# WeiZhang1988/YDORBSLAM

Measured on AMD Instinct MI355X. Metric: ORB extract+match Mkeypoints/sec, higher is better.
Workload: dtype u8

## Files before the change

ydorbslam_amd/csrc/ba_kernels.hip.h:

```cpp
#pragma once
#include <hip/hip_runtime.h>
#include <stdint.h>
#include "g2o_math.hip.h"

#pragma clang fp contract(off)

namespace ydorb {
namespace ba {

using g2o::R; using g2o::V3; using g2o::Q4;
using g2o::add; using g2o::cross; using g2o::scale; using g2o::qrot; using g2o::qmul; using g2o::qToR; using g2o::rToQ; using g2o::qnormalize;
using g2o::huber; using g2o::block_sums; using g2o::block_sum1; using g2o::dense_solve; using g2o::lambda_init; using g2o::lm_judge;

struct Cam { R fx, fy, cx, cy, bf; };

struct EdgeSoA {
  const int* pose;
  const int* pidx;
  const int* pt;
  const R* meas;
  const R* info;
  const uint8_t* robust;
  int n;
};
// ... 271 lines not shown

__device__ __forceinline__ int pair_bucket(int i1, int i2) { return i2 * (i2 + 1) / 2 + i1; }

__global__ __launch_bounds__(256) void k_pair_count(EdgeSoA Ed, const int* __restrict__ ptStart, int nL, int* __restrict__ cnt) {
  const int l = blockIdx.x * 256 + threadIdx.x;
  if (l >= nL) return;
  for (int a = ptStart[l]; a < ptStart[l + 1]; a++) {
    const int i1 = Ed.pidx[a];
    if (i1 < 0) continue;
    for (int b = a; b < ptStart[l + 1]; b++) {
      const int i2 = Ed.pidx[b];
      if (i2 >= 0) atomicAdd(&cnt[pair_bucket(i1, i2)], 1);
    }
  }
}
__global__ __launch_bounds__(256) void k_excl_scan(const int* __restrict__ in, int n, int* __restrict__ out) {
  __shared__ int wsum[4];
  __shared__ int carryS;
  const int lane = threadIdx.x & 63, wv = threadIdx.x >> 6;
  if (threadIdx.x == 0) carryS = 0;
  __syncthreads();
  for (int c0 = 0; c0 < n; c0 += 256) {
    const int i = c0 + threadIdx.x;
    const int v = i < n ? in[i] : 0;
    int x = v;
#pragma unroll
    for (int d = 1; d < 64; d <<= 1) { const int y = __shfl_up(x, d, 64); if (lane >= d) x += y; }
    if (lane == 63) wsum[wv] = x;
    __syncthreads();
    int off = carryS;
    for (int j = 0; j < wv; j++) off += wsum[j];
    if (i < n) out[i] = off + x - v;
    __syncthreads();
    if (threadIdx.x == 0) carryS += wsum[0] + wsum[1] + wsum[2] + wsum[3];
    __syncthreads();
  }
  if (threadIdx.x == 0) out[n] = carryS;
}
__global__ __launch_bounds__(256) void k_pair_fill(EdgeSoA Ed, const int* __restrict__ ptStart, int nL, int* __restrict__ cursor,
                                                   int2* __restrict__ items) {
  const int l = blockIdx.x * 256 + threadIdx.x;
  if (l >= nL) return;
  for (int a = ptStart[l]; a < ptStart[l + 1]; a++) {
    const int i1 = Ed.pidx[a];
    if (i1 < 0) continue;
    for (int b = a; b < ptStart[l + 1]; b++) {
      const int i2 = Ed.pidx[b];
      if (i2 >= 0) items[atomicAdd(&cursor[pair_bucket(i1, i2)], 1)] = make_int2(a, b);
    }
  }
}
constexpr int kSortCap = 2048;
// ... 857 lines not shown
```

ydorbslam_amd/csrc/ba_solver.hip:

```cpp
#include <hip/hip_runtime.h>
#include <chrono>

#include <algorithm>
#include <string>
#include <thread>
#include <atomic>
#include <cmath>
#include <cstring>
#include <limits>
#include <mutex>
#include <numeric>
#include <optional>
#include <vector>

#include "../../include/ydorb/c_api.h"
#include "ba_kernels.hip.h"
#include "ba_pairs.h"
#include "ba_skyline.hip.h"
#include "host_buffers.h"
#include "lm_schedule.h"
#include "ydorb_host.h"

using namespace ydorb;
using namespace ydorb::ba;

namespace {

enum { PH_ERR = 0, PH_BUILD, PH_SCHUR, PH_SOLVE, PH_UPDATE, PH_COUNT };

struct Sys {
  std::vector<int> act; int nL = 0, nPf = 0, Ea = 0, n = 0, nb = 0, nBlkE = 0, nBuckets = 0, nPoseEdges = 0; size_t nItems = 0;
  bool sky = false;
  sky::Plan plan;
  size_t envDoubles() const { return 36 * (size_t)plan.envBlocks; }
};
static_assert(bapairs::kDenseMaxRows == kCholSolveMaxN, "ba_pairs.h states the dense limit for the host-only plan");

struct StatePtrs { double *poses[2], *pts[2]; };
size_t layState(int K, int NP, void* base, StatePtrs& st) {
  Carve a(base);
  for (int i = 0; i < 2; i++) { a.take(st.poses[i], (size_t)7 * K); a.take(st.pts[i], (size_t)3 * NP); }
  return a.L.bytes;
}

struct SkyPtrs { int *pairRow, *pairI1, *pairI2, *perm, *first, *colRows; long long *pairDst, *rowOff, *colStart, *colBlk; };
struct UpPtrs { int *ePose, *ePidx, *ePt, *eLm, *ptStart, *poseStart, *ptOf, *poseEdges, *poseOf; double *eMeas, *eInfo; uint8_t* eRobust; SkyPtrs k; };
size_t layUp(const Sys& Y, void* base, UpPtrs& u) {
  Carve a(base);
  const size_t Ea = Y.Ea;
  a.take(u.ePose, Ea); a.take(u.ePidx, Ea); a.take(u.ePt, Ea); a.take(u.eLm, Ea); a.take(u.eMeas, 3 * Ea); a.take(u.eInfo, Ea); a.take(u.eRobust, Ea);
  a.take(u.ptStart, Y.nL + 1); a.take(u.poseStart, Y.nPf + 1); a.take(u.ptOf, Y.nL); a.take(u.poseEdges, Y.nPoseEdges); a.take(u.poseOf, Y.nPf);
  u.k = SkyPtrs{};
  if (Y.sky) {
    const size_t nB = Y.nBuckets, nF = Y.nPf, nCol = Y.plan.colRows.size();
    a.take(u.k.pairRow, nF + 1); a.take(u.k.pairI1, nB); a.take(u.k.pairI2, nB); a.take(u.k.pairDst, nB); a.take(u.k.perm, nF); a.take(u.k.first, nF);
    a.take(u.k.rowOff, nF + 1); a.take(u.k.colStart, nF + 1); a.take(u.k.colRows, nCol); a.take(u.k.colBlk, nCol);
  }
  return a.L.bytes;
}

struct WorkPtrs {
  double *eInfo0, *err, *partial, *Hll, *bl, *Hpl, *BD, *Hpp, *S, *diagInv, *diagL, *Dinv, *db, *xp, *xl, *yv, *skyW, *scal;
  uint8_t* eOutlier;
  int *status, *pairCnt, *pairStart, *pairCursor;
  int2 *pairA, *pairB;
  double* bp(const Sys& Y) const { return Hpp + (size_t)36 * Y.nPf; }
// ... 15 lines not shown
struct PosePtrs { int *start, *inl, *trials; double *poses, *X, *meas, *info, *err, *chi; uint8_t *flags, *outlier; };
size_t layPose(int n, size_t E, void* base, PosePtrs& q) {
  Carve a(base);
  a.take(q.start, n + 1); a.take(q.poses, (size_t)7 * n); a.take(q.X, 3 * E); a.take(q.meas, 3 * E); a.take(q.info, E);
  a.take(q.err, 3 * E); a.take(q.flags, E); a.take(q.outlier, E); a.take(q.inl, n); a.take(q.chi, (size_t)4 * n); a.take(q.trials, n);
  return a.L.bytes;
}

struct SolveMem {
  int device = -1;
  hipStream_t stream = nullptr;
  Mem state, up, work;
  StatePtrs st{};
  UpPtrs u{};
  WorkPtrs w{};
  PinnedMem hStage;
  int stage(size_t bytes) { return bytes <= hStage.cap ? YDORB_OK : hStage.alloc(bytes + bytes / 4 + 4096); }
  void releaseBuffers() { for (Mem* m : {&state, &up, &work, static_cast<Mem*>(&hStage)}) m->release(); }
};

struct Ctx {
  SolveMem mem;
  Mem pose;
  hipEvent_t ev[2 * PH_COUNT + 2]{};
  PinnedMem hPin;
  void releaseBuffers() { mem.releaseBuffers(); pose.release(); }
};
constexpr int kCtxPool = 8;
std::mutex g_mu[16][kCtxPool];
Ctx g_ctx[16][kCtxPool];
std::mutex g_pick;

// ... 12 lines not shown
    HIPCHK(hipStreamCreateWithFlags(&c.mem.stream, hipStreamNonBlocking));
    for (auto& e : c.ev) HIPCHK(hipEventCreate(&e));
    return c.hPin.alloc(sizeof(double) * 16);
  };
  if (!c.mem.stream && init() != YDORB_OK) return nullptr;
  return &c;
}

struct Run {
  SolveMem* c;
  const YdBaProblem* P;
  const YdBaOptions* O;
  YdBaResult* res;
  int cur = 0;
  bool noRobust = false;
  Cam cam;
  bool phaseTimes = false;
  double phaseMs[PH_COUNT] = {0, 0, 0, 0, 0};
  bool pending[PH_COUNT] = {false, false, false, false, false};
  Sys sys;
  hipEvent_t* ev = nullptr;
  double* hPin = nullptr;
  LmSchedule lm;
  const YdBaSolverOptions* SO = nullptr;
  YdBaSolverInfo* info = nullptr;
  bool stopped() const { return LmSchedule::raised(P->stop); }
};

int tooWideForSolve(int n) {
  set_error("reduced camera system of %d rows is wider than the solve kernel's LDS (max %d)", n, kCholSolveMaxN);
// ... 37 lines not shown
}

int allreduce(Run& R_, void* d_buf, int64_t count, int op) {
  const YdBaOptions* O = R_.O;
  if (!O->allreduce || O->world <= 1) return YDORB_OK;
  if (count > O->comm_doubles || !O->d_comm_buf) { set_error("BA comm buffer too small (%lld doubles needed)", (long long)count); return YDORB_ERR_CAPACITY; }
  HIPCHK(hipMemcpyAsync(O->d_comm_buf, d_buf, sizeof(double) * count, hipMemcpyDeviceToDevice, R_.c->stream));
  HIPCHK(hipStreamSynchronize(R_.c->stream));
  if (O->allreduce(O->allreduce_user, O->d_comm_buf, count, op) != 0) { set_error("BA all-reduce callback failed"); return YDORB_ERR_HIP; }
  HIPCHK(hipMemcpyAsync(d_buf, O->d_comm_buf, sizeof(double) * count, hipMemcpyDeviceToDevice, R_.c->stream));
  return YDORB_OK;
}

static bool g_trace = getenv("YDORB_BA_TRACE") != nullptr && getenv("YDORB_BA_TRACE")[0] == '1';
static std::chrono::steady_clock::time_point g_t0;
static void trace(const char* what) {
  if (!g_trace) return;
  fprintf(stderr, "[ba %8.3f ms] %s\n", std::chrono::duration<double, std::milli>(std::chrono::steady_clock::now() - g_t0).count(), what);
}

struct PhaseTimer {
  Run& r; int ph; hipEvent_t a, b; bool on;
  PhaseTimer(Run& r_, int ph_) : r(r_), ph(ph_), a(r_.ev[2 * ph_]), b(r_.ev[2 * ph_ + 1]), on(r_.phaseTimes) {
    if (!on) return;
    collect(r_, ph_);
    (void)hipEventRecord(a, r.c->stream);
  }
  void stop() { if (on) { (void)hipEventRecord(b, r.c->stream); on = false; r.pending[ph] = true; } }
  static void collect(Run& r_, int ph_) {
    if (!r_.pending[ph_]) return;
    float ms = 0;
    if (hipEventSynchronize(r_.ev[2 * ph_ + 1]) == hipSuccess && hipEventElapsedTime(&ms, r_.ev[2 * ph_], r_.ev[2 * ph_ + 1]) == hipSuccess)
      r_.phaseMs[ph_] += ms;
    r_.pending[ph_] = false;
  }
};

int prepareStage(Run& R_, bool reuse) {
  SolveMem& c = *R_.c;
  const YdBaProblem& P = *R_.P;
  const YdBaOptions& O = *R_.O;
  hipStream_t s = c.stream;
  const int K = P.n_poses, NP = P.n_points, E = P.n_edges;
  trace("optimize: begin");
  Sys& Y = R_.sys;
  auto prepare = [&]() -> int {
    std::vector<int> act;
    for (int e = 0; e < E; e++) act.push_back(e);
    if (act.empty()) { Y.Ea = 0; return YDORB_OK; }
    std::vector<int> poseIdx(K, -1), ptIdx(NP, -1), poseOf, ptOf;
    {
      std::vector<uint8_t> pu(K, 0), qu(NP, 0);
      for (int e : act) { pu[P.edge_pose[e]] = 1; qu[P.edge_point[e]] = 1; }
      for (int k = 0; k < K; k++) if (pu[k] && !P.pose_fixed[k]) { poseIdx[k] = (int)poseOf.size(); poseOf.push_back(k); }
      for (int p = 0; p < NP; p++) if (qu[p]) { ptIdx[p] = (int)ptOf.size(); ptOf.push_back(p); }
    }
    const int nL = (int)ptOf.size(), Ea = (int)act.size();
    if (O.world > 1) {
      poseOf.clear();
      for (int k = 0; k < K; k++) { poseIdx[k] = -1; if (!P.pose_fixed[k]) { poseIdx[k] = (int)poseOf.size(); poseOf.push_back(k); } }
    }
    const int nPf = (int)poseOf.size();
    {
      std::vector<int> start(nL + 1, 0), sorted(Ea);
      for (int e : act) start[ptIdx[P.edge_point[e]] + 1]++;
      for (int l = 0; l < nL; l++) start[l + 1] += start[l];
      std::vector<int> fill(start.begin(), start.end() - 1);
      for (int e : act) sorted[fill[ptIdx[P.edge_point[e]]]++] = e;
      auto after = [&](int x, int y) {
        const int px = poseIdx[P.edge_pose[x]], py = poseIdx[P.edge_pose[y]];
        return px != py ? px > py : P.edge_pose[x] > P.edge_pose[y];
      };
      for (int l = 0; l < nL; l++)
        for (int a = start[l] + 1; a < start[l + 1]; a++) {
          const int e = sorted[a];
          int b = a - 1;
          while (b >= start[l] && after(sorted[b], e)) { sorted[b + 1] = sorted[b]; b--; }
          sorted[b + 1] = e;
          if (b >= start[l] && P.edge_pose[sorted[b]] == P.edge_pose[e]) {
            set_error("edges %d and %d are both the observation of point %d by pose %d", sorted[b], e, P.edge_point[e], P.edge_pose[e]);
            return YDORB_ERR_INVALID_ARG;
          }
        }
      act.swap(sorted);
    }
    std::vector<int> hPose(Ea), hPidx(Ea), hPt(Ea), hLm(Ea), hPtStart(nL + 1, 0), hPoseStart(nPf + 1, 0), hPoseEdges;
    std::vector<double> hMeas((size_t)3 * Ea), hInfo(Ea);
    std::vector<uint8_t> hRobust(Ea);
    for (int i = 0; i < Ea; i++) {
      const int e = act[i];
      hPose[i] = P.edge_pose[e]; hPidx[i] = poseIdx[P.edge_pose[e]]; hPt[i] = P.edge_point[e]; hLm[i] = ptIdx[P.edge_point[e]];
      for (int d = 0; d < 3; d++) hMeas[3 * i + d] = P.edge_meas[3 * e + d];
      hInfo[i] = P.edge_inv_sigma2[e];
      hRobust[i] = R_.noRobust ? 0 : 1;
      hPtStart[hLm[i] + 1]++;
      if (hPidx[i] >= 0) hPoseStart[hPidx[i] + 1]++;
    }
    for (int l = 0; l < nL; l++) hPtStart[l + 1] += hPtStart[l];
    for (int i = 0; i < nPf; i++) hPoseStart[i + 1] += hPoseStart[i];
    hPoseEdges.resize(hPoseStart[nPf]);
    {
      std::vector<int> fill(hPoseStart.begin(), hPoseStart.end() - 1);
      for (int i = 0; i < Ea; i++) if (hPidx[i] >= 0) hPoseEdges[fill[hPidx[i]]++] = i;
    }
    Sys Z;
    Z.nL = nL; Z.nPf = nPf; Z.Ea = Ea; Z.nPoseEdges = (int)hPoseEdges.size();
    Z.n = std::max(NB, (6 * nPf + NB - 1) / NB * NB); Z.nb = Z.n / NB;
    Z.nBlkE = (Ea + 255) / 256;
    Z.nBuckets = (int)std::min<long long>((long long)nPf * (nPf + 1) / 2, std::numeric_limits<int>::max());
    for (int l = 0; l < nL; l++) {
      size_t m = 0;
      for (int i = hPtStart[l]; i < hPtStart[l + 1]; i++) m += hPidx[i] >= 0;
      Z.nItems += m * (m + 1) / 2;
    }
    bapairs::PairList pairs;
    std::vector<int64_t> pairDst;
    {
      int rc = chooseSolver(R_.SO, O.world, nPf, [&] { return bapairs::buildPairs(nPf, nL, hPtStart.data(), hPidx.data()); }, true, pairs, Z.plan, Z.sky, R_.info);
      if (rc) return rc;
      if (Z.sky) {
        Z.n = 6 * nPf; Z.nb = 0; Z.nBuckets = (int)pairs.buckets();
        pairDst = bapairs::bucketDestinations(pairs, Z.plan);
      }
    }
    trace("optimize: host ordering done");
    const size_t upBytes = layUp(Z, nullptr, c.u);
    int rc;
    if ((rc = c.stage(upBytes)) || (rc = c.up.ensure(upBytes)) || (rc = c.work.ensure(layWork(Z, nullptr, c.w)))) return rc;
    layUp(Z, c.up.p, c.u);
    layWork(Z, c.work.p, c.w);
    const UpPtrs& u = c.u;
    const WorkPtrs& w = c.w;
    {
      auto up = [&](const void* dst, const void* src, size_t bytes) {
        if (bytes) memcpy(c.hStage.as<uint8_t>() + (static_cast<const uint8_t*>(dst) - c.up.as<uint8_t>()), src, bytes);
      };
      auto upv = [&](const auto* dst, const auto& vec) { up(dst, vec.data(), sizeof(vec[0]) * vec.size()); };
      upv(u.ePose, hPose); upv(u.ePidx, hPidx); upv(u.ePt, hPt); upv(u.eLm, hLm); upv(u.eMeas, hMeas); upv(u.eInfo, hInfo);
      upv(u.eRobust, hRobust); upv(u.ptStart, hPtStart); upv(u.poseStart, hPoseStart); upv(u.ptOf, ptOf);
      upv(u.poseEdges, hPoseEdges); upv(u.poseOf, poseOf);
      if (Z.sky) {
        const sky::Plan& K = Z.plan;
        upv(u.k.pairRow, pairs.rowStart); upv(u.k.pairI1, pairs.i1); upv(u.k.pairI2, pairs.i2); upv(u.k.pairDst, pairDst); upv(u.k.perm, K.perm);
        upv(u.k.first, K.first); upv(u.k.rowOff, K.rowOff); upv(u.k.colStart, K.colStart); upv(u.k.colRows, K.colRows); upv(u.k.colBlk, K.colBlk);
      }
      HIPCHK(hipMemcpyAsync(c.up.p, c.hStage.p, upBytes, hipMemcpyHostToDevice, s));
      HIPCHK(hipMemcpyAsync(w.eInfo0, u.eInfo, sizeof(double) * Ea, hipMemcpyDeviceToDevice, s));
      HIPCHK(hipMemsetAsync(w.err, 0, sizeof(double) * 3 * Ea, s));
    }
    trace("optimize: uploads enqueued");
    if (Z.nBuckets > 0) {
      const int nBuckets = Z.nBuckets;
      EdgeSoA Ed{u.ePose, u.ePidx, u.ePt, u.eMeas, u.eInfo, u.eRobust, Ea};
      HIPCHK(hipMemsetAsync(w.pairCnt, 0, sizeof(int) * (nBuckets + 1), s));
      if (Z.sky) hipLaunchKernelGGL(k_sky_pair_count, dim3((nL + 255) / 256), dim3(256), 0, s, Ed, u.ptStart, nL, u.k.pairRow, u.k.pairI1, w.pairCnt);
      else hipLaunchKernelGGL(k_pair_count, dim3((nL + 255) / 256), dim3(256), 0, s, Ed, u.ptStart, nL, w.pairCnt);
      hipLaunchKernelGGL(k_excl_scan, dim3(1), dim3(256), 0, s, w.pairCnt, nBuckets, w.pairStart);
      HIPCHK(hipMemcpyAsync(w.pairCursor, w.pairStart, sizeof(int) * (nBuckets + 1), hipMemcpyDeviceToDevice, s));
      if (Z.sky) hipLaunchKernelGGL(k_sky_pair_fill, dim3((nL + 255) / 256), dim3(256), 0, s, Ed, u.ptStart, nL, u.k.pairRow, u.k.pairI1, w.pairCursor, w.pairA);
      else hipLaunchKernelGGL(k_pair_fill, dim3((nL + 255) / 256), dim3(256), 0, s, Ed, u.ptStart, nL, w.pairCursor, w.pairA);
      hipLaunchKernelGGL(k_pair_sort, dim3((nBuckets + 3) / 4), dim3(256), 0, s, w.pairStart, nBuckets, w.pairA, w.pairB);
    }
    HIPCHK(hipStreamSynchronize(s));
    Z.act.swap(act);
    Y = std::move(Z);
    return YDORB_OK;
  };
  int rc;
  if (!reuse || Y.Ea == 0) {
    if ((rc = prepare())) return rc;
  }
  if (Y.Ea == 0) return YDORB_OK;
  HIPCHK(hipMemcpyAsync(c.st.poses[R_.cur ^ 1], c.st.poses[R_.cur], sizeof(double) * 7 * K, hipMemcpyDeviceToDevice, s));
  HIPCHK(hipMemcpyAsync(c.st.pts[R_.cur ^ 1], c.st.pts[R_.cur], sizeof(double) * 3 * NP, hipMemcpyDeviceToDevice, s));
  if (!Y.sky) HIPCHK(hipMemsetAsync(c.w.S, 0, sizeof(double) * ((size_t)Y.n * Y.n + Y.n + (size_t)Y.nb * NB * NB), s));
  return YDORB_OK;
}

int launchSchur(Run& R_, double lambda, double contrib) {
// ... 41 lines not shown
  const YdBaOptions& O = *R_.O;
  hipStream_t s = c.stream;
  const Sys& Y = R_.sys;
  if (Y.Ea == 0) return YDORB_OK;
  const int nL = Y.nL, nPf = Y.nPf, Ea = Y.Ea, n = Y.n, nBlkE = Y.nBlkE;
  const UpPtrs& u = c.u;
  const WorkPtrs& w = c.w;
  double* const* poses = c.st.poses;
  double* const* pts = c.st.pts;
  double *dHpp = w.Hpp, *dbp = w.bp(Y), *dS = w.S;
  EdgeSoA Ed{u.ePose, u.ePidx, u.ePt, u.eMeas, u.eInfo, u.eRobust, Ea};
  const double dM = O.delta_mono, dSt = O.delta_stereo;
  double* hscal = R_.hPin;
  const bool multi = O.world > 1 && O.allreduce;

  auto computeChi2 = [&](int buf, bool withStatus) -> int {
    PhaseTimer t(R_, PH_ERR);
    hipLaunchKernelGGL(k_errors, dim3(nBlkE), dim3(256), 0, s, Ed, poses[buf], pts[buf], R_.cam, dM, dSt, w.err, w.partial);
    hipLaunchKernelGGL(k_sum_partials, dim3(1), dim3(256), 0, s, w.partial, nBlkE, w.scal, 0, withStatus ? w.status : nullptr);
    t.stop();
    if (multi) { int r2 = allreduce(R_, w.scal, 1, 0); if (r2) return r2; }
    HIPCHK(hipMemcpyAsync(hscal, w.scal, sizeof(double) * 8, hipMemcpyDeviceToHost, s));
    HIPCHK(hipStreamSynchronize(s));
    return YDORB_OK;
  };

  trace("optimize: pair buckets enqueued");
  const double& lambda = lm.lambda;
  for (bool more = lm.firstIteration(R_.P->stop); more;) {
    if (lm.needChi2()) {
      if ((rc = computeChi2(R_.cur, false))) return rc;
      lm.setChi2(hscal[0]);
    }
    {
      PhaseTimer t(R_, PH_BUILD);
      hipLaunchKernelGGL(k_build_points, dim3((nL + 127) / 128), dim3(128), 0, s, Ed, u.ptStart, nL, poses[R_.cur], pts[R_.cur], R_.cam, dM, dSt, w.err, w.Hll, w.bl, w.Hpl);
      if (nPf)
        hipLaunchKernelGGL(k_build_poses, dim3(nPf), dim3(256), 0, s, Ed, u.poseStart, u.poseEdges, poses[R_.cur], pts[R_.cur], R_.cam, dM, dSt, w.err, dHpp, dbp);
// ... 73 lines not shown
  return YDORB_OK;
}

int beginSolve(Run& R_) {
  SolveMem& c = *R_.c;
  const YdBaProblem* P = R_.P;
  const YdBaOptions& O = *R_.O;
  const int K = P->n_poses, NP = P->n_points;
  int rc;
  R_.noRobust = (O.flags & YDORB_BA_NO_ROBUST) != 0;
  R_.phaseTimes = (O.flags & YDORB_BA_PHASE_TIMES) != 0;
  R_.cam = Cam{P->fx, P->fy, P->cx, P->cy, P->bf};
  R_.lm.begin(O, R_.res);
  if ((rc = c.state.ensure(layState(K, NP, nullptr, c.st)))) return rc;
  layState(K, NP, c.state.p, c.st);
  {
    std::vector<double> hp(P->poses, P->poses + (size_t)7 * K);
    for (int k = 0; k < K; k++) {
      double* q = &hp[7 * k + 3];
      if (q[3] < 0) for (int d = 0; d < 4; d++) q[d] = -q[d];
      const double nrm = sqrt(q[0] * q[0] + q[1] * q[1] + q[2] * q[2] + q[3] * q[3]);
      for (int d = 0; d < 4; d++) q[d] /= nrm;
    }
    HIPCHK(hipMemcpyAsync(c.st.poses[0], hp.data(), sizeof(double) * 7 * K, hipMemcpyHostToDevice, c.stream));
    HIPCHK(hipStreamSynchronize(c.stream));
  }
  HIPCHK(hipMemcpyAsync(c.st.pts[0], P->points, sizeof(double) * 3 * NP, hipMemcpyHostToDevice, c.stream));
  return YDORB_OK;
}

int launchCull(Run& R_, int final) {
  SolveMem& c = *R_.c;
  const YdBaOptions& O = *R_.O;
  const int Ea = R_.sys.Ea;
  if (Ea == 0) return YDORB_OK;
  hipLaunchKernelGGL(k_cull, dim3((Ea + 255) / 256), dim3(256), 0, c.stream, c.u.ePose, c.u.ePt, c.u.eMeas, Ea, c.w.eInfo0, c.w.err,
                     c.st.poses[R_.cur], c.st.pts[R_.cur], O.chi2_mono, O.chi2_stereo, final, c.u.eInfo, c.u.eRobust, c.w.eOutlier);
  HIPCHK(hipGetLastError());
  return YDORB_OK;
}

int endSolve(Run& R_) {
  SolveMem& c = *R_.c;
  const YdBaProblem* P = R_.P;
  const Sys& Y = R_.sys;
  int rc = launchCull(R_, 1);
  if (rc) return rc;
  uint8_t* outlier = R_.res->edge_outlier;
  const size_t bPoses = sizeof(double) * 7 * P->n_poses, bPts = sizeof(double) * 3 * P->n_points, oPts = (bPoses + 255) & ~(size_t)255,
               oOut = oPts + ((bPts + 255) & ~(size_t)255);
  if ((rc = c.stage(oOut + Y.Ea))) return rc;
  if (outlier && Y.Ea) HIPCHK(hipMemcpyAsync(c.hStage.as<uint8_t>() + oOut, c.w.eOutlier, Y.Ea, hipMemcpyDeviceToHost, c.stream));
  HIPCHK(hipMemcpyAsync(c.hStage.as<uint8_t>(), c.st.poses[R_.cur], bPoses, hipMemcpyDeviceToHost, c.stream));
  HIPCHK(hipMemcpyAsync(c.hStage.as<uint8_t>() + oPts, c.st.pts[R_.cur], bPts, hipMemcpyDeviceToHost, c.stream));
  HIPCHK(hipStreamSynchronize(c.stream));
  memcpy(P->poses, c.hStage.as<uint8_t>(), bPoses);
  memcpy(P->points, c.hStage.as<uint8_t>() + oPts, bPts);
  if (outlier) for (int i = 0; i < Y.Ea; i++) outlier[Y.act[i]] = c.hStage.as<uint8_t>()[oOut + i];
  if (R_.stopped()) R_.res->stopped = 1;
  return YDORB_OK;
}

struct Job {
  SolveMem mem;
  BaDev dev{};
  YdBaOptions O;
  std::optional<Run> run;
  bool needBuild = false;
  bool done = false;
  bool pendingEnd = false;
  int rc = YDORB_OK;
  std::string errText;
};
// ... 52 lines not shown
        if (!R_.lm.handOver(R_.P->stop)) { X.pendingEnd = X.done = true; return; }
        if ((r = launchCull(R_, 0))) { fail(j, r); return; }
      }
      if ((r = prepareStage(R_, R_.lm.stage == 2))) { fail(j, r); return; }
      if (R_.sys.Ea == 0) continue;
      if (R_.sys.n > kCholSolveMaxN) { fail(j, tooWideForSolve(R_.sys.n)); return; }
      fillDev(X, X.dev, B.dDev.as<BaDev>(), dScalAll + (size_t)8 * j, dStatusAll + (size_t)2 * j);
      if (R_.lm.firstIteration(R_.P->stop)) { X.needBuild = true; return; }
    }
  };
  auto spread = [&](auto fn) {
    const int nt = std::max(1, std::min(n, kSetupThreads));
    std::atomic<int> next{0};
    auto worker = [&](int t) {
      (void)hipSetDevice(Oin.device);
      for (int j = next.fetch_add(1); j < n; j = next.fetch_add(1)) fn(j, B.setupStreams[t]);
    };
    std::vector<std::thread> pool;
    for (int t = 1; t < nt; t++) pool.emplace_back(worker, t);
    worker(0);
    for (std::thread& th : pool) th.join();
    for (int j = 0; j < n; j++) if (J[j]->rc != YDORB_OK && !J[j]->errText.empty()) set_error("%s", J[j]->errText.c_str());
  };

  while ((int)B.setupStreams.size() < std::min(n, kSetupThreads)) {
    hipStream_t st = nullptr;
    HIPCHK(hipStreamCreateWithFlags(&st, hipStreamNonBlocking));
    B.setupStreams.push_back(st);
  }
  spread([&](int j, hipStream_t st) {
    Job& X = *J[j];
// ... 3 lines not shown
    int r = checkProblem(&probs[j], &Oin, &res[j], &X.O);
    const YdBaProblem* P = &probs[j];
    if (!r) {
      if (P->stop && *P->stop) { res[j].stopped = 1; X.done = true; return; }
      if (P->n_edges == 0 || P->n_poses == 0 || P->n_points == 0) { X.done = true; return; }
      X.mem.device = Oin.device; X.mem.stream = st;
      X.run.emplace(Run{&X.mem, P, &X.O, &res[j]});
      r = beginSolve(*X.run);
    }
    if (!r) {
      nextStage(j, false);
      r = X.rc;
    }
    if (r) { X.errText = ydorb_last_error(); fail(j, r); }
    if (hipStreamSynchronize(st) != hipSuccess && !r) { X.errText = "hipStreamSynchronize failed"; fail(j, YDORB_ERR_HIP); }
    X.mem.stream = s;
  });
  trace("batch: set-up done");

  auto maxOver = [&](auto fn) { int m = 0; for (int j = 0; j < n; j++) if (!J[j]->done) m = std::max(m, fn(J[j]->run->sys)); return m; };
  auto rounds = [&]() -> int {
    while (true) {
      bool any = false;
      for (int j = 0; j < n; j++) any = any || !J[j]->done;
      if (!any) break;
      trace("batch: round begins");
      bool anyBuild = false, anyChi = false, anyDiag = false;
      for (int j = 0; j < n; j++) {
        Job& X = *J[j];
        BaDev& D = hDevA[j];
// ... 150 lines not shown
  int rc = checkProblem(P, optIn, res, &O);
  if (rc) return rc;
  const int K = P->n_poses, NP = P->n_points, E = P->n_edges;
  if (P->stop && *P->stop) { res->stopped = 1; return YDORB_OK; }
  if (E == 0 || K == 0 || NP == 0) return YDORB_OK;
  if ((rc = require_device(O.device))) return rc;
  g_t0 = std::chrono::steady_clock::now();
  trace("solve: begin");
  std::unique_lock<std::mutex> lock;
  Ctx* ctx = acquireCtx(O.device, lock);
  if (!ctx) return YDORB_ERR_HIP;
  Ctx& c = *ctx;
  Run R_{&c.mem, P, &O, res};
  R_.ev = c.ev; R_.hPin = c.hPin.as<double>();
  R_.SO = &SO; R_.info = info;
  if ((rc = beginSolve(R_))) return rc;
  trace("solve: state uploaded");
  hipEvent_t t0 = c.ev[2 * PH_COUNT], t1 = c.ev[2 * PH_COUNT + 1];
  HIPCHK(hipEventRecord(t0, c.mem.stream));

  for (;;) {
    if ((rc = optimize(R_))) return rc;
    if (!R_.lm.handOver(P->stop)) break;
    if ((rc = launchCull(R_, 0))) return rc;
    trace("solve: depths read");
  }
  HIPCHK(hipEventRecord(t1, c.mem.stream));
  if ((rc = endSolve(R_))) return rc;
  (void)hipEventElapsedTime(&res->ms_total, t0, t1);
  trace("solve: results read back");
  res->ms_errors = (float)R_.phaseMs[PH_ERR]; res->ms_build = (float)R_.phaseMs[PH_BUILD]; res->ms_schur = (float)R_.phaseMs[PH_SCHUR];
  res->ms_solve = (float)R_.phaseMs[PH_SOLVE]; res->ms_update = (float)R_.phaseMs[PH_UPDATE];
  return YDORB_OK;
}

int ydorb_pose_optimize(const YdPoseBatch* B, uint8_t* outlier, int32_t* n_inliers, double* chi2_log, int32_t* trials) {
  if (!B || B->n_frames < 0 || (B->n_frames && (!B->edge_start || !B->poses || !n_inliers)) || B->device < 0 || B->device >= 16) {
    set_error("invalid pose batch");
    return YDORB_ERR_INVALID_ARG;
  }
  const int n = B->n_frames;
  if (n == 0) return YDORB_OK;
  if (B->edge_start[0] != 0) { set_error("edge_start[0] must be 0"); return YDORB_ERR_INVALID_ARG; }
// ... 155 lines not shown
  if (!S_out || !bs_out || !x_out || !solved) { set_error("null argument"); return YDORB_ERR_INVALID_ARG; }
  const YdBaSolverOptions SO = sopt ? *sopt : YdBaSolverOptions{YDORB_BA_SOLVER_AUTO, YDORB_ESS_ORDER_SMALLER, 0};
  YdBaResult res{};
  YdBaOptions O;
  int rc = checkProblem(P, optIn, &res, &O);
  if (rc) return rc;
  if (P->n_edges == 0 || O.world > 1) { set_error("reduced system: needs edges and a single rank"); return YDORB_ERR_INVALID_ARG; }
  if ((rc = require_device(O.device))) return rc;
  std::unique_lock<std::mutex> lock;
  Ctx* ctx = acquireCtx(O.device, lock);
  if (!ctx) return YDORB_ERR_HIP;
  Ctx& c = *ctx;
  Run R_{&c.mem, P, &O, &res};
  R_.ev = c.ev; R_.hPin = c.hPin.as<double>();
  R_.SO = &SO;
  if ((rc = beginSolve(R_))) return rc;
  if ((rc = prepareStage(R_, false))) return rc;
  const Sys& Y = R_.sys;
  const int F = Y.nPf, n6 = 6 * F;
  if (Y.Ea == 0 || F == 0) { set_error("reduced system: no free pose"); return YDORB_ERR_INVALID_ARG; }
  if (n6 > 4096) { set_error("reduced system: %d rows, at most 4096 are expanded", n6); return YDORB_ERR_UNSUPPORTED; }
  hipStream_t s = c.mem.stream;
  const UpPtrs& u = c.mem.u;
  const WorkPtrs& w = c.mem.w;
  EdgeSoA Ed{u.ePose, u.ePidx, u.ePt, u.eMeas, u.eInfo, u.eRobust, Y.Ea};
  const double *poses = c.mem.st.poses[R_.cur], *pts = c.mem.st.pts[R_.cur];
  hipLaunchKernelGGL(k_errors, dim3(Y.nBlkE), dim3(256), 0, s, Ed, poses, pts, R_.cam, O.delta_mono, O.delta_stereo, w.err, w.partial);
  hipLaunchKernelGGL(k_build_points, dim3((Y.nL + 127) / 128), dim3(128), 0, s, Ed, u.ptStart, Y.nL, poses, pts, R_.cam, O.delta_mono, O.delta_stereo, w.err, w.Hll, w.bl, w.Hpl);
  hipLaunchKernelGGL(k_build_poses, dim3(F), dim3(256), 0, s, Ed, u.poseStart, u.poseEdges, poses, pts, R_.cam, O.delta_mono, O.delta_stereo, w.err, w.Hpp, w.bp(Y));
  if ((rc = launchSchur(R_, lambda, 1.0))) return rc;
// ... 88 lines not shown
```

Baseline: 178.6.

## Overlap BA host ordering with structure upload and drop redundant host staging syncs

Moves BA problem ordering into a reusable scratch planner and writes the upload image directly into pinned staging. It splits the upload so the structure arrays and pair-bucket kernels are enqueued before the host writes measurement values. It also removes a blocking sync and copy in state upload, and fuses the pair-cursor copy into the scan kernel. The aim is to overlap host prep with device work and cut allocations, at the cost of extra syncs when staging is reallocated and more complex buffer lifetime handling.

```diff
diff --git a/ydorbslam_amd/csrc/ba_kernels.hip.h b/ydorbslam_amd/csrc/ba_kernels.hip.h
--- a/ydorbslam_amd/csrc/ba_kernels.hip.h
+++ b/ydorbslam_amd/csrc/ba_kernels.hip.h
@@ -309,7 +309,7 @@
     }
   }
 }
-__global__ __launch_bounds__(256) void k_excl_scan(const int* __restrict__ in, int n, int* __restrict__ out) {
+__global__ __launch_bounds__(256) void k_excl_scan(const int* __restrict__ in, int n, int* __restrict__ out, int* __restrict__ out2) {
   __shared__ int wsum[4];
   __shared__ int carryS;
   const int lane = threadIdx.x & 63, wv = threadIdx.x >> 6;
@@ -325,12 +325,12 @@
     __syncthreads();
     int off = carryS;
     for (int j = 0; j < wv; j++) off += wsum[j];
-    if (i < n) out[i] = off + x - v;
+    if (i < n) out[i] = out2[i] = off + x - v;
     __syncthreads();
     if (threadIdx.x == 0) carryS += wsum[0] + wsum[1] + wsum[2] + wsum[3];
     __syncthreads();
   }
-  if (threadIdx.x == 0) out[n] = carryS;
+  if (threadIdx.x == 0) out[n] = out2[n] = carryS;
 }
 __global__ __launch_bounds__(256) void k_pair_fill(EdgeSoA Ed, const int* __restrict__ ptStart, int nL, int* __restrict__ cursor,
                                                    int2* __restrict__ items) {
diff --git a/ydorbslam_amd/csrc/ba_order.h b/ydorbslam_amd/csrc/ba_order.h
--- /dev/null
+++ b/ydorbslam_amd/csrc/ba_order.h
@@ -0,0 +1,115 @@
+#pragma once
+#include <stdint.h>
+#include <stdio.h>
+
+#include <string>
+#include <vector>
+
+namespace ydorb {
+namespace baorder {
+
+struct Graph {
+  int K = 0, NP = 0, E = 0;
+  const int32_t *edgePose = nullptr, *edgePoint = nullptr;
+  const uint8_t* poseFixed = nullptr;
+  bool allUnfixedFree = false;
+};
+
+struct Scratch {
+  std::vector<int> act, poseIdx, ptIdx, poseOf, ptOf, ptStart;
+  int nL = 0, nPf = 0, Ea = 0, nPoseEdges = 0;
+  size_t nItems = 0;
+  std::vector<int> fill;
+  std::vector<uint8_t> used;
+};
+
+struct Arrays {
+  int *ePose, *ePidx, *ePt, *eLm, *ptStart, *poseStart, *ptOf, *poseEdges, *poseOf;
+  double *eMeas, *eInfo;
+  uint8_t* eRobust;
+};
+
+inline bool plan(const Graph& G, Scratch& S, std::string& err) {
+  const int K = G.K, NP = G.NP, E = G.E;
+  S.nL = S.nPf = S.Ea = S.nPoseEdges = 0; S.nItems = 0;
+  S.poseIdx.resize(K); S.ptIdx.resize(NP); S.poseOf.resize(K); S.ptOf.resize(NP);
+  S.used.resize((size_t)K + NP);
+  for (size_t i = 0; i < (size_t)K + NP; i++) S.used[i] = 0;
+  uint8_t *pu = S.used.data(), *qu = pu + K;
+  for (int e = 0; e < E; e++) { pu[G.edgePose[e]] = 1; qu[G.edgePoint[e]] = 1; }
+  int nPf = 0, nL = 0;
+  for (int k = 0; k < K; k++) {
+    const bool free = !G.poseFixed[k] && (G.allUnfixedFree || pu[k]);
+    S.poseIdx[k] = free ? nPf : -1;
+    if (free) S.poseOf[nPf++] = k;
+  }
+  for (int p = 0; p < NP; p++) {
+    S.ptIdx[p] = qu[p] ? nL : -1;
+    if (qu[p]) S.ptOf[nL++] = p;
+  }
+  S.nPf = nPf; S.nL = nL;
+  S.act.resize(E); S.ptStart.resize((size_t)nL + 1); S.fill.resize((size_t)(nL > nPf ? nL : nPf) + 1);
+  int* start = S.ptStart.data();
+  int* sorted = S.act.data();
+  for (int l = 0; l <= nL; l++) start[l] = 0;
+  for (int e = 0; e < E; e++) start[S.ptIdx[G.edgePoint[e]] + 1]++;
+  for (int l = 0; l < nL; l++) { start[l + 1] += start[l]; S.fill[l] = start[l]; }
+  for (int e = 0; e < E; e++) sorted[S.fill[S.ptIdx[G.edgePoint[e]]]++] = e;
+  for (int l = 0; l < nL; l++) {
+    size_t m = 0;
+    for (int a = start[l]; a < start[l + 1]; a++) {
+      const int e = sorted[a], pe = G.edgePose[e], ie = S.poseIdx[pe];
+      int b = a - 1;
+      for (; b >= start[l]; b--) {
+        const int pb = G.edgePose[sorted[b]], ib = S.poseIdx[pb];
+        if (!(ib != ie ? ib > ie : pb > pe)) break;
+        sorted[b + 1] = sorted[b];
+      }
+      sorted[b + 1] = e;
+      if (b >= start[l] && G.edgePose[sorted[b]] == pe) {
+        char text[160];
+        snprintf(text, sizeof(text), "edges %d and %d are both the observation of point %d by pose %d", sorted[b], e, G.edgePoint[e], pe);
+        err = text;
+        return false;
+      }
+      m += ie >= 0;
+    }
+    S.nPoseEdges += (int)m;
+    S.nItems += m * (m + 1) / 2;
+  }
+  S.Ea = E;
+  return true;
+}
+
+inline void emitStructure(const Graph& G, Scratch& S, const Arrays& A) {
+  const int Ea = S.Ea, nL = S.nL, nPf = S.nPf;
+  for (int i = 0; i <= nPf; i++) A.poseStart[i] = 0;
+  for (int i = 0; i < Ea; i++) {
+    const int e = S.act[i], k = G.edgePose[e], p = G.edgePoint[e], pi = S.poseIdx[k];
+    A.ePose[i] = k; A.ePidx[i] = pi; A.ePt[i] = p; A.eLm[i] = S.ptIdx[p];
+    if (pi >= 0) A.poseStart[pi + 1]++;
+  }
+  for (int l = 0; l <= nL; l++) A.ptStart[l] = S.ptStart[l];
+  for (int l = 0; l < nL; l++) A.ptOf[l] = S.ptOf[l];
+  for (int i = 0; i < nPf; i++) { A.poseStart[i + 1] += A.poseStart[i]; S.fill[i] = A.poseStart[i]; A.poseOf[i] = S.poseOf[i]; }
+  for (int i = 0; i < Ea; i++) {
+    const int pi = A.ePidx[i];
+    if (pi >= 0) A.poseEdges[S.fill[pi]++] = i;
+  }
+}
+inline void emitValues(const Scratch& S, const double* meas, const double* info, bool robust, const Arrays& A) {
+  const int Ea = S.Ea;
+  for (int i = 0; i < Ea; i++) {
+    const size_t e = (size_t)S.act[i];
+    for (int d = 0; d < 3; d++) A.eMeas[3 * (size_t)i + d] = meas[3 * e + d];
+    A.eInfo[i] = info[e];
+    A.eRobust[i] = robust ? 1 : 0;
+  }
+}
+inline void emit(const Graph& G, Scratch& S, const double* meas, const double* info, bool robust, const Arrays& A) {
+  emitStructure(G, S, A);
+  emitValues(S, meas, info, robust, A);
+}
+
+}
+}
diff --git a/ydorbslam_amd/csrc/ba_solver.hip b/ydorbslam_amd/csrc/ba_solver.hip
--- a/ydorbslam_amd/csrc/ba_solver.hip
+++ b/ydorbslam_amd/csrc/ba_solver.hip
@@ -15,6 +15,7 @@
 
 #include "../../include/ydorb/c_api.h"
 #include "ba_kernels.hip.h"
+#include "ba_order.h"
 #include "ba_pairs.h"
 #include "ba_skyline.hip.h"
 #include "host_buffers.h"
@@ -29,7 +30,7 @@
 enum { PH_ERR = 0, PH_BUILD, PH_SCHUR, PH_SOLVE, PH_UPDATE, PH_COUNT };
 
 struct Sys {
-  std::vector<int> act; int nL = 0, nPf = 0, Ea = 0, n = 0, nb = 0, nBlkE = 0, nBuckets = 0, nPoseEdges = 0; size_t nItems = 0;
+  int nL = 0, nPf = 0, Ea = 0, n = 0, nb = 0, nBlkE = 0, nBuckets = 0, nPoseEdges = 0; size_t nItems = 0;
   bool sky = false;
   sky::Plan plan;
   size_t envDoubles() const { return 36 * (size_t)plan.envBlocks; }
@@ -44,12 +45,15 @@
 }
 
 struct SkyPtrs { int *pairRow, *pairI1, *pairI2, *perm, *first, *colRows; long long *pairDst, *rowOff, *colStart, *colBlk; };
-struct UpPtrs { int *ePose, *ePidx, *ePt, *eLm, *ptStart, *poseStart, *ptOf, *poseEdges, *poseOf; double *eMeas, *eInfo; uint8_t* eRobust; SkyPtrs k; };
+struct UpPtrs { int *ePose, *ePidx, *ePt, *eLm, *ptStart, *poseStart, *ptOf, *poseEdges, *poseOf; double *eMeas, *eInfo; uint8_t* eRobust; SkyPtrs k; size_t valuesOff; };
 size_t layUp(const Sys& Y, void* base, UpPtrs& u) {
   Carve a(base);
   const size_t Ea = Y.Ea;
-  a.take(u.ePose, Ea); a.take(u.ePidx, Ea); a.take(u.ePt, Ea); a.take(u.eLm, Ea); a.take(u.eMeas, 3 * Ea); a.take(u.eInfo, Ea); a.take(u.eRobust, Ea);
+  a.take(u.ePose, Ea); a.take(u.ePidx, Ea); a.take(u.ePt, Ea); a.take(u.eLm, Ea);
   a.take(u.ptStart, Y.nL + 1); a.take(u.poseStart, Y.nPf + 1); a.take(u.ptOf, Y.nL); a.take(u.poseEdges, Y.nPoseEdges); a.take(u.poseOf, Y.nPf);
+  a.take(u.eMeas, 3 * Ea);
+  u.valuesOff = reinterpret_cast<uintptr_t>(u.eMeas) - a.base;
+  a.take(u.eInfo, Ea); a.take(u.eRobust, Ea);
   u.k = SkyPtrs{};
   if (Y.sky) {
     const size_t nB = Y.nBuckets, nF = Y.nPf, nCol = Y.plan.colRows.size();
@@ -95,8 +99,15 @@
   StatePtrs st{};
   UpPtrs u{};
   WorkPtrs w{};
+  baorder::Scratch order;
   PinnedMem hStage;
-  int stage(size_t bytes) { return bytes <= hStage.cap ? YDORB_OK : hStage.alloc(bytes + bytes / 4 + 4096); }
+  size_t upOff = 0;
+  int stage(size_t bytes) {
+    if (bytes <= hStage.cap) return YDORB_OK;
+    if (stream) HIPCHK(hipStreamSynchronize(stream));
+    return hStage.alloc(bytes + bytes / 4 + 4096);
+  }
+  void settle() { if (stream) (void)hipStreamSynchronize(stream); }
   void releaseBuffers() { for (Mem* m : {&state, &up, &work, static_cast<Mem*>(&hStage)}) m->release(); }
 };
 
@@ -139,6 +150,7 @@
   YdBaResult* res;
   int cur = 0;
   bool noRobust = false;
+  bool splitUpload = false;
   Cam cam;
   bool phaseTimes = false;
   double phaseMs[PH_COUNT] = {0, 0, 0, 0, 0};
@@ -206,9 +218,12 @@
 
 static bool g_trace = getenv("YDORB_BA_TRACE") != nullptr && getenv("YDORB_BA_TRACE")[0] == '1';
 static std::chrono::steady_clock::time_point g_t0;
+static thread_local int t_traceThread = -1;
 static void trace(const char* what) {
   if (!g_trace) return;
-  fprintf(stderr, "[ba %8.3f ms] %s\n", std::chrono::duration<double, std::milli>(std::chrono::steady_clock::now() - g_t0).count(), what);
+  const double ms = std::chrono::duration<double, std::milli>(std::chrono::steady_clock::now() - g_t0).count();
+  if (t_traceThread < 0) fprintf(stderr, "[ba %8.3f ms] %s\n", ms, what);
+  else fprintf(stderr, "[ba %8.3f ms] t%02d %s\n", ms, t_traceThread, what);
 }
 
 struct PhaseTimer {
@@ -237,78 +252,28 @@
   trace("optimize: begin");
   Sys& Y = R_.sys;
   auto prepare = [&]() -> int {
-    std::vector<int> act;
-    for (int e = 0; e < E; e++) act.push_back(e);
-    if (act.empty()) { Y.Ea = 0; return YDORB_OK; }
-    std::vector<int> poseIdx(K, -1), ptIdx(NP, -1), poseOf, ptOf;
+    if (E == 0) { Y.Ea = 0; return YDORB_OK; }
+    baorder::Scratch& Q = c.order;
+    const baorder::Graph G{K, NP, E, P.edge_pose, P.edge_point, P.pose_fixed, O.world > 1};
     {
-      std::vector<uint8_t> pu(K, 0), qu(NP, 0);
-      for (int e : act) { pu[P.edge_pose[e]] = 1; qu[P.edge_point[e]] = 1; }
-      for (int k = 0; k < K; k++) if (pu[k] && !P.pose_fixed[k]) { poseIdx[k] = (int)poseOf.size(); poseOf.push_back(k); }
-      for (int p = 0; p < NP; p++) if (qu[p]) { ptIdx[p] = (int)ptOf.size(); ptOf.push_back(p); }
-    }
-    const int nL = (int)ptOf.size(), Ea = (int)act.size();
-    if (O.world > 1) {
-      poseOf.clear();
-      for (int k = 0; k < K; k++) { poseIdx[k] = -1; if (!P.pose_fixed[k]) { poseIdx[k] = (int)poseOf.size(); poseOf.push_back(k); } }
-    }
-    const int nPf = (int)poseOf.size();
-    {
-      std::vector<int> start(nL + 1, 0), sorted(Ea);
-      for (int e : act) start[ptIdx[P.edge_point[e]] + 1]++;
-      for (int l = 0; l < nL; l++) start[l + 1] += start[l];
-      std::vector<int> fill(start.begin(), start.end() - 1);
-      for (int e : act) sorted[fill[ptIdx[P.edge_point[e]]]++] = e;
-      auto after = [&](int x, int y) {
-        const int px = poseIdx[P.edge_pose[x]], py = poseIdx[P.edge_pose[y]];
-        return px != py ? px > py : P.edge_pose[x] > P.edge_pose[y];
-      };
-      for (int l = 0; l < nL; l++)
-        for (int a = start[l] + 1; a < start[l + 1]; a++) {
-          const int e = sorted[a];
-          int b = a - 1;
-          while (b >= start[l] && after(sorted[b], e)) { sorted[b + 1] = sorted[b]; b--; }
-          sorted[b + 1] = e;
-          if (b >= start[l] && P.edge_pose[sorted[b]] == P.edge_pose[e]) {
-            set_error("edges %d and %d are both the observation of point %d by pose %d", sorted[b], e, P.edge_point[e], P.edge_pose[e]);
-            return YDORB_ERR_INVALID_ARG;
-          }
-        }
-      act.swap(sorted);
-    }
-    std::vector<int> hPose(Ea), hPidx(Ea), hPt(Ea), hLm(Ea), hPtStart(nL + 1, 0), hPoseStart(nPf + 1, 0), hPoseEdges;
-    std::vector<double> hMeas((size_t)3 * Ea), hInfo(Ea);
-    std::vector<uint8_t> hRobust(Ea);
-    for (int i = 0; i < Ea; i++) {
-      const int e = act[i];
-      hPose[i] = P.edge_pose[e]; hPidx[i] = poseIdx[P.edge_pose[e]]; hPt[i] = P.edge_point[e]; hLm[i] = ptIdx[P.edge_point[e]];
-      for (int d = 0; d < 3; d++) hMeas[3 * i + d] = P.edge_meas[3 * e + d];
-      hInfo[i] = P.edge_inv_sigma2[e];
-      hRobust[i] = R_.noRobust ? 0 : 1;
-      hPtStart[hLm[i] + 1]++;
-      if (hPidx[i] >= 0) hPoseStart[hPidx[i] + 1]++;
-    }
-    for (int l = 0; l < nL; l++) hPtStart[l + 1] += hPtStart[l];
-    for (int i = 0; i < nPf; i++) hPoseStart[i + 1] += hPoseStart[i];
-    hPoseEdges.resize(hPoseStart[nPf]);
-    {
-      std::vector<int> fill(hPoseStart.begin(), hPoseStart.end() - 1);
-      for (int i = 0; i < Ea; i++) if (hPidx[i] >= 0) hPoseEdges[fill[hPidx[i]]++] = i;
-    }
+      std::string err;
+      if (!baorder::plan(G, Q, err)) { set_error("%s", err.c_str()); return YDORB_ERR_INVALID_ARG; }
+    }
+    const int nL = Q.nL, nPf = Q.nPf, Ea = Q.Ea;
     Sys Z;
-    Z.nL = nL; Z.nPf = nPf; Z.Ea = Ea; Z.nPoseEdges = (int)hPoseEdges.size();
+    Z.nL = nL; Z.nPf = nPf; Z.Ea = Ea; Z.nPoseEdges = Q.nPoseEdges; Z.nItems = Q.nItems;
     Z.n = std::max(NB, (6 * nPf + NB - 1) / NB * NB); Z.nb = Z.n / NB;
     Z.nBlkE = (Ea + 255) / 256;
     Z.nBuckets = (int)std::min<long long>((long long)nPf * (nPf + 1) / 2, std::numeric_limits<int>::max());
-    for (int l = 0; l < nL; l++) {
-      size_t m = 0;
-      for (int i = hPtStart[l]; i < hPtStart[l + 1]; i++) m += hPidx[i] >= 0;
-      Z.nItems += m * (m + 1) / 2;
-    }
     bapairs::PairList pairs;
     std::vector<int64_t> pairDst;
     {
-      int rc = chooseSolver(R_.SO, O.world, nPf, [&] { return bapairs::buildPairs(nPf, nL, hPtStart.data(), hPidx.data()); }, true, pairs, Z.plan, Z.sky, R_.info);
+      auto makePairs = [&] {
+        std::vector<int> pidx(Ea);
+        for (int i = 0; i < Ea; i++) pidx[i] = Q.poseIdx[P.edge_pose[Q.act[i]]];
+        return bapairs::buildPairs(nPf, nL, Q.ptStart.data(), pidx.data());
+      };
+      int rc = chooseSolver(R_.SO, O.world, nPf, makePairs, true, pairs, Z.plan, Z.sky, R_.info);
       if (rc) return rc;
       if (Z.sky) {
         Z.n = 6 * nPf; Z.nb = 0; Z.nBuckets = (int)pairs.buckets();
@@ -318,43 +283,51 @@
     trace("optimize: host ordering done");
     const size_t upBytes = layUp(Z, nullptr, c.u);
     int rc;
-    if ((rc = c.stage(upBytes)) || (rc = c.up.ensure(upBytes)) || (rc = c.work.ensure(layWork(Z, nullptr, c.w)))) return rc;
+    if ((rc = c.stage(c.upOff + upBytes)) || (rc = c.up.ensure(upBytes)) || (rc = c.work.ensure(layWork(Z, nullptr, c.w)))) return rc;
     layUp(Z, c.up.p, c.u);
     layWork(Z, c.work.p, c.w);
     const UpPtrs& u = c.u;
     const WorkPtrs& w = c.w;
-    {
-      auto up = [&](const void* dst, const void* src, size_t bytes) {
-        if (bytes) memcpy(c.hStage.as<uint8_t>() + (static_cast<const uint8_t*>(dst) - c.up.as<uint8_t>()), src, bytes);
-      };
-      auto upv = [&](const auto* dst, const auto& vec) { up(dst, vec.data(), sizeof(vec[0]) * vec.size()); };
-      upv(u.ePose, hPose); upv(u.ePidx, hPidx); upv(u.ePt, hPt); upv(u.eLm, hLm); upv(u.eMeas, hMeas); upv(u.eInfo, hInfo);
-      upv(u.eRobust, hRobust); upv(u.ptStart, hPtStart); upv(u.poseStart, hPoseStart); upv(u.ptOf, ptOf);
-      upv(u.poseEdges, hPoseEdges); upv(u.poseOf, poseOf);
-      if (Z.sky) {
-        const sky::Plan& K = Z.plan;
-        upv(u.k.pairRow, pairs.rowStart); upv(u.k.pairI1, pairs.i1); upv(u.k.pairI2, pairs.i2); upv(u.k.pairDst, pairDst); upv(u.k.perm, K.perm);
-        upv(u.k.first, K.first); upv(u.k.rowOff, K.rowOff); upv(u.k.colStart, K.colStart); upv(u.k.colRows, K.colRows); upv(u.k.colBlk, K.colBlk);
-      }
-      HIPCHK(hipMemcpyAsync(c.up.p, c.hStage.p, upBytes, hipMemcpyHostToDevice, s));
-      HIPCHK(hipMemcpyAsync(w.eInfo0, u.eInfo, sizeof(double) * Ea, hipMemcpyDeviceToDevice, s));
-      HIPCHK(hipMemsetAsync(w.err, 0, sizeof(double) * 3 * Ea, s));
-    }
-    trace("optimize: uploads enqueued");
-    if (Z.nBuckets > 0) {
+    auto pairBuckets = [&]() -> int {
+      if (Z.nBuckets == 0) return YDORB_OK;
       const int nBuckets = Z.nBuckets;
       EdgeSoA Ed{u.ePose, u.ePidx, u.ePt, u.eMeas, u.eInfo, u.eRobust, Ea};
       HIPCHK(hipMemsetAsync(w.pairCnt, 0, sizeof(int) * (nBuckets + 1), s));
       if (Z.sky) hipLaunchKernelGGL(k_sky_pair_count, dim3((nL + 255) / 256), dim3(256), 0, s, Ed, u.ptStart, nL, u.k.pairRow, u.k.pairI1, w.pairCnt);
       else hipLaunchKernelGGL(k_pair_count, dim3((nL + 255) / 256), dim3(256), 0, s, Ed, u.ptStart, nL, w.pairCnt);
-      hipLaunchKernelGGL(k_excl_scan, dim3(1), dim3(256), 0, s, w.pairCnt, nBuckets, w.pairStart);
-      HIPCHK(hipMemcpyAsync(w.pairCursor, w.pairStart, sizeof(int) * (nBuckets + 1), hipMemcpyDeviceToDevice, s));
+      hipLaunchKernelGGL(k_excl_scan, dim3(1), dim3(256), 0, s, w.pairCnt, nBuckets, w.pairStart, w.pairCursor);
       if (Z.sky) hipLaunchKernelGGL(k_sky_pair_fill, dim3((nL + 255) / 256), dim3(256), 0, s, Ed, u.ptStart, nL, u.k.pairRow, u.k.pairI1, w.pairCursor, w.pairA);
       else hipLaunchKernelGGL(k_pair_fill, dim3((nL + 255) / 256), dim3(256), 0, s, Ed, u.ptStart, nL, w.pairCursor, w.pairA);
       hipLaunchKernelGGL(k_pair_sort, dim3((nBuckets + 3) / 4), dim3(256), 0, s, w.pairStart, nBuckets, w.pairA, w.pairB);
-    }
-    HIPCHK(hipStreamSynchronize(s));
-    Z.act.swap(act);
+      return YDORB_OK;
+    };
+    {
+      uint8_t* image = c.hStage.as<uint8_t>() + c.upOff;
+      UpPtrs h;
+      layUp(Z, image, h);
+      const baorder::Arrays A{h.ePose, h.ePidx, h.ePt, h.eLm, h.ptStart, h.poseStart, h.ptOf, h.poseEdges, h.poseOf, h.eMeas, h.eInfo, h.eRobust};
+      const size_t first = R_.splitUpload && !Z.sky ? h.valuesOff : 0;
+      baorder::emitStructure(G, Q, A);
+      if (first) {
+        trace("optimize: structure written");
+        HIPCHK(hipMemcpyAsync(c.up.p, image, first, hipMemcpyHostToDevice, s));
+        if ((rc = pairBuckets())) return rc;
+      }
+      baorder::emitValues(Q, P.edge_meas, P.edge_inv_sigma2, !R_.noRobust, A);
+      if (Z.sky) {
+        auto upv = [](auto* dst, const auto& vec) { if (!vec.empty()) memcpy(dst, vec.data(), sizeof(vec[0]) * vec.size()); };
+        const sky::Plan& K = Z.plan;
+        upv(h.k.pairRow, pairs.rowStart); upv(h.k.pairI1, pairs.i1); upv(h.k.pairI2, pairs.i2); upv(h.k.pairDst, pairDst); upv(h.k.perm, K.perm);
+        upv(h.k.first, K.first); upv(h.k.rowOff, K.rowOff); upv(h.k.colStart, K.colStart); upv(h.k.colRows, K.colRows); upv(h.k.colBlk, K.colBlk);
+      }
+      trace("optimize: staging written");
+      HIPCHK(hipMemcpyAsync(c.up.as<uint8_t>() + first, image + first, upBytes - first, hipMemcpyHostToDevice, s));
+      if (!first && (rc = pairBuckets())) return rc;
+      HIPCHK(hipMemcpyAsync(w.eInfo0, u.eInfo, sizeof(double) * Ea, hipMemcpyDeviceToDevice, s));
+      HIPCHK(hipMemsetAsync(w.err, 0, sizeof(double) * 3 * Ea, s));
+    }
+    trace("optimize: uploads enqueued");
+    HIPCHK(hipGetLastError());
     Y = std::move(Z);
     return YDORB_OK;
   };
@@ -426,6 +399,7 @@
   double* hscal = R_.hPin;
   const bool multi = O.world > 1 && O.allreduce;
 
+  bool readBack = false;
   auto computeChi2 = [&](int buf, bool withStatus) -> int {
     PhaseTimer t(R_, PH_ERR);
     hipLaunchKernelGGL(k_errors, dim3(nBlkE), dim3(256), 0, s, Ed, poses[buf], pts[buf], R_.cam, dM, dSt, w.err, w.partial);
@@ -434,6 +408,7 @@
     if (multi) { int r2 = allreduce(R_, w.scal, 1, 0); if (r2) return r2; }
     HIPCHK(hipMemcpyAsync(hscal, w.scal, sizeof(double) * 8, hipMemcpyDeviceToHost, s));
     HIPCHK(hipStreamSynchronize(s));
+    if (!readBack) { readBack = true; trace("optimize: first read-back"); }
     return YDORB_OK;
   };
 
@@ -537,18 +512,24 @@
   R_.lm.begin(O, R_.res);
   if ((rc = c.state.ensure(layState(K, NP, nullptr, c.st)))) return rc;
   layState(K, NP, c.state.p, c.st);
+  const size_t bPoses = sizeof(double) * 7 * K, bPts = sizeof(double) * 3 * NP, oPts = (bPoses + 255) & ~(size_t)255;
+  c.upOff = oPts + ((bPts + 255) & ~(size_t)255);
   {
-    std::vector<double> hp(P->poses, P->poses + (size_t)7 * K);
-    for (int k = 0; k < K; k++) {
-      double* q = &hp[7 * k + 3];
-      if (q[3] < 0) for (int d = 0; d < 4; d++) q[d] = -q[d];
-      const double nrm = sqrt(q[0] * q[0] + q[1] * q[1] + q[2] * q[2] + q[3] * q[3]);
-      for (int d = 0; d < 4; d++) q[d] /= nrm;
-    }
-    HIPCHK(hipMemcpyAsync(c.st.poses[0], hp.data(), sizeof(double) * 7 * K, hipMemcpyHostToDevice, c.stream));
-    HIPCHK(hipStreamSynchronize(c.stream));
-  }
-  HIPCHK(hipMemcpyAsync(c.st.pts[0], P->points, sizeof(double) * 3 * NP, hipMemcpyHostToDevice, c.stream));
+    Sys most;
+    most.Ea = most.nPoseEdges = P->n_edges; most.nL = NP; most.nPf = K;
+    UpPtrs unused;
+    if ((rc = c.stage(c.upOff + layUp(most, nullptr, unused)))) return rc;
+  }
+  double* hp = c.hStage.as<double>();
+  memcpy(hp, P->poses, bPoses);
+  for (int k = 0; k < K; k++) {
+    double* q = &hp[7 * k + 3];
+    if (q[3] < 0) for (int d = 0; d < 4; d++) q[d] = -q[d];
+    const double nrm = sqrt(q[0] * q[0] + q[1] * q[1] + q[2] * q[2] + q[3] * q[3]);
+    for (int d = 0; d < 4; d++) q[d] /= nrm;
+  }
+  memcpy(c.hStage.as<uint8_t>() + oPts, P->points, bPts);
+  HIPCHK(hipMemcpyAsync(c.st.poses[0], hp, oPts + bPts, hipMemcpyHostToDevice, c.stream));
   return YDORB_OK;
 }
 
@@ -579,7 +560,11 @@
   HIPCHK(hipStreamSynchronize(c.stream));
   memcpy(P->poses, c.hStage.as<uint8_t>(), bPoses);
   memcpy(P->points, c.hStage.as<uint8_t>() + oPts, bPts);
-  if (outlier) for (int i = 0; i < Y.Ea; i++) outlier[Y.act[i]] = c.hStage.as<uint8_t>()[oOut + i];
+  if (outlier) {
+    const int* act = c.order.act.data();
+    const uint8_t* flags = c.hStage.as<uint8_t>() + oOut;
+    for (int i = 0; i < Y.Ea; i++) outlier[act[i]] = flags[i];
+  }
   if (R_.stopped()) R_.res->stopped = 1;
   return YDORB_OK;
 }
@@ -662,7 +647,9 @@
     std::atomic<int> next{0};
     auto worker = [&](int t) {
       (void)hipSetDevice(Oin.device);
+      t_traceThread = t;
       for (int j = next.fetch_add(1); j < n; j = next.fetch_add(1)) fn(j, B.setupStreams[t]);
+      t_traceThread = -1;
     };
     std::vector<std::thread> pool;
     for (int t = 1; t < nt; t++) pool.emplace_back(worker, t);
@@ -696,6 +683,7 @@
     }
     if (r) { X.errText = ydorb_last_error(); fail(j, r); }
     if (hipStreamSynchronize(st) != hipSuccess && !r) { X.errText = "hipStreamSynchronize failed"; fail(j, YDORB_ERR_HIP); }
+    trace("batch: member set up");
     X.mem.stream = s;
   });
   trace("batch: set-up done");
@@ -876,19 +864,23 @@
   Run R_{&c.mem, P, &O, res};
   R_.ev = c.ev; R_.hPin = c.hPin.as<double>();
   R_.SO = &SO; R_.info = info;
-  if ((rc = beginSolve(R_))) return rc;
-  trace("solve: state uploaded");
+  R_.splitUpload = true;
   hipEvent_t t0 = c.ev[2 * PH_COUNT], t1 = c.ev[2 * PH_COUNT + 1];
-  HIPCHK(hipEventRecord(t0, c.mem.stream));
-
-  for (;;) {
-    if ((rc = optimize(R_))) return rc;
-    if (!R_.lm.handOver(P->stop)) break;
-    if ((rc = launchCull(R_, 0))) return rc;
-    trace("solve: depths read");
-  }
-  HIPCHK(hipEventRecord(t1, c.mem.stream));
-  if ((rc = endSolve(R_))) return rc;
+  auto solve = [&]() -> int {
+    int r;
+    if ((r = beginSolve(R_))) return r;
+    trace("solve: state upload enqueued");
+    HIPCHK(hipEventRecord(t0, c.mem.stream));
+    for (;;) {
+      if ((r = optimize(R_))) return r;
+      if (!R_.lm.handOver(P->stop)) break;
+      if ((r = launchCull(R_, 0))) return r;
+      trace("solve: depths read");
+    }
+    HIPCHK(hipEventRecord(t1, c.mem.stream));
+    return endSolve(R_);
+  };
+  if ((rc = solve())) { c.mem.settle(); return rc; }
   (void)hipEventElapsedTime(&res->ms_total, t0, t1);
   trace("solve: results read back");
   res->ms_errors = (float)R_.phaseMs[PH_ERR]; res->ms_build = (float)R_.phaseMs[PH_BUILD]; res->ms_schur = (float)R_.phaseMs[PH_SCHUR];
@@ -1074,6 +1066,7 @@
   Run R_{&c.mem, P, &O, &res};
   R_.ev = c.ev; R_.hPin = c.hPin.as<double>();
   R_.SO = &SO;
+  struct Settle { SolveMem& m; ~Settle() { m.settle(); } } settleOnReturn{c.mem};
   if ((rc = beginSolve(R_))) return rc;
   if ((rc = prepareStage(R_, false))) return rc;
   const Sys& Y = R_.sys;
```

Measured after the change: 177.2. No clear change (-0.8%).
